# HKUST-Aerial-Robotics/Omni-swarm

Hardware: AMD Instinct MI355X
Metric: keyframes/sec (4x fisheye 600x480) + p50 loop-match ms @ 100k-frame DB (higher is better)
Workload: dtype f16

## Files before the change

### omni-swarm_amd/csrc/config.h

```cpp
#pragma once
#include "common.h"

namespace omni {

enum CfgId {
    CFG_CONV_V1 = 0, CFG_RS_TRN, CFG_DET16, CFG_SP_SPARSE_DESC, CFG_SP_SPARSE_DA, CFG_SP_FUSED_CAND, CFG_SP_SPLIT_DB, CFG_SP_MASK_SKIP, CFG_SP_MASK_SKIP_SPLIT, CFG_SP_MASK_RECT, CFG_SPLIT_FUSE1A, CFG_SPLIT_WINO,
    CFG_SPLIT_TRN, CFG_CONV_XCD, CFG_SP_PROFILE_MASK, CFG_PP_U8, CFG_PP_TRACE, CFG_PP_DBG, CFG_RS_TRACE, CFG_SPLIT_TRACE, CFG_SPLIT_DBG, CFG_WINO_TRACE, CFG_ROCTX,
    CFG_VLAD_BIG, CFG_VLAD_STEM_FUSE, CFG_VLAD_UNFUSED, CFG_VLAD_MFMA, CFG_VLAD_SBLOCK, CFG_VLAD_MBLOCK_PX, CFG_VLAD_MFMA_PX, CFG_VLAD_FC_MFMA, CFG_VLAD_MBLOCK_CPW,
    CFG_VLAD_SB_LDSPAD, CFG_VLAD_SB_PERSIST, CFG_VLAD_SB_TRACE, CFG_VLAD_SB_DBG, CFG_VLAD_MASK_SKIP,
    CFG_SCAN_ROWS_MIN, CFG_MQ_ROT, CFG_MQ_MIN, CFG_INDEX_MIRROR, CFG_INDEX_MIRROR_MIN_ROWS, CFG_INDEX_CERT_FAIL,
    CFG_GEOMETRY_THREADS, CFG_MESSAGE_THREADS, CFG_GEOMETRY_ASYNC, CFG_DETECTOR_ASYNC, CFG_PIPELINE_ONE_STREAM, CFG_PIPELINE_FIFO, CFG_PIPELINE_UNIT_PLAN,
    CFG_HW_QUEUES,
    CFG_RCCL_LIB,
    CFG_COUNT
};
enum CfgClass {
    CFG_VARIANT = 0,
    CFG_TUNING = 1,
    CFG_DEBUG = 2,
    CFG_TEST = 3,
    CFG_STRING = 4
};
struct CfgOption { const char* env; int def, lo, hi; int cls; const char* doc; };
extern const CfgOption kCfgOptions[CFG_COUNT];

struct Config {
    int v[CFG_COUNT];
    int operator[](CfgId i) const { return v[i]; }
};
int config_resolve(Config* out);
const Config& config_process();
int config_option_now(CfgId i);

}
```

### omni-swarm_amd/csrc/config.hip

```cpp
#include "config.h"

#include <atomic>
#include <cerrno>
#include <climits>
#include <cstdlib>

namespace omni {

const CfgOption kCfgOptions[CFG_COUNT] = {
    {"OMNI_CONV_V1", 0, 0, 3, CFG_VARIANT, "fp16 3x3 layers: 0 = production (conv1a fused into the ping-pong conv1b, register-stationary cin=128); 1 = generic kernel, 2 = persistent LDS-DMA kernel, "
                                           "3 = ping-pong without the conv1a fusion -- 1-3 exist only in the test build of the library (lib_test/)"},
    {"OMNI_RS_TRN", -1, -1, 1, CFG_VARIANT, "register-stationary kernel of the unpooled cin=128 fp16 layers: tile orientation, -1 = the one with fewer tiles, 0 = plain, 1 = transposed"},
    {"OMNI_DET16", 1, 0, 1, CFG_VARIANT, "detector head of the fp16 and OMNI_PREC_SPLIT paths on v_mfma_f32_32x32x16_f16 with split (hi, lo) operands (0: the exact-f32 MFMA kernel)"},
    {"OMNI_SP_SPARSE_DESC", 1, 0, 1, CFG_VARIANT, "convDb + descriptor norm only at the cells around the key points (0: dense descriptor map)"},
    {"OMNI_SP_SPARSE_DA", 1, 0, 1, CFG_VARIANT, "convDa only at those cells too (fp16 and OMNI_PREC_SPLIT; 0: dense convDa)"},
    {"OMNI_SP_FUSED_CAND", 1, 0, 1, CFG_VARIANT, "getKeyPoints' threshold inside the detector head's epilogue + window masks from the candidate list (0: sp_cand_kernel re-reads the heat map)"},
    {"OMNI_SP_SPLIT_DB", 1, 0, 1, CFG_VARIANT, "OMNI_PREC_SPLIT: convDb + descriptor norm at the key points' cells with split (hi, lo) operands on the fp16 matrix cores (0: exact-f32 MFMA convolution)"},
    {"OMNI_SP_MASK_SKIP", 1, 0, 1, CFG_VARIANT, "fp16: the tile rows inside the image-independent band of the fisheye mask are left out of the tile walk (0: every tile)"},
    {"OMNI_SP_MASK_SKIP_SPLIT", 1, 0, 1, CFG_VARIANT, "the same for OMNI_PREC_SPLIT"},
    {"OMNI_SP_MASK_RECT", 0, 0, 1, CFG_TEST, "1: a masked pass leaves out only the rectangle of tiles where the output is one constant vector, filled by broadcasting that vector "
                                             "(what was skipped before the band: the A/B reference, same results)"},
    {"OMNI_SPLIT_FUSE1A", 1, 0, 1, CFG_VARIANT, "OMNI_PREC_SPLIT: conv1a built inside the conv1b kernel from the u8 image (0: separate exact-f32 conv1a pass)"},
    {"OMNI_SPLIT_WINO", 7, 0, 15, CFG_VARIANT, "OMNI_PREC_SPLIT: the cin = 64 layers as Winograd F(2x2,3x3) kernels with split operands (conv_wino.hip), bit 0 = conv1b (with the conv1a "
                                                "fusion), 1 = conv2a, 2 = conv2b, 3 = conv3a (off by default: same time as the direct kernel, profiles/r06g); 0: the direct kernels of conv_split.hip"},
    {"OMNI_SPLIT_TRN", -1, -1, 1, CFG_VARIANT, "OMNI_PREC_SPLIT cin=128 kernel: tile orientation, as OMNI_RS_TRN"},
    {"OMNI_CONV_XCD", 1, 0, 1, CFG_VARIANT, "persistent convolution kernels derive (cout group, tile walk) from an XCD-aware block id: the cout groups of a pixel tile and its neighbours "
                                           "share one L2 (0: plain blockIdx; process-wide, same results either way)"},
    {"OMNI_SP_PROFILE_MASK", 0, 0, 1, CFG_TUNING, "omni_sp_profile times the stages with the fisheye mask on (what the key-frame pipeline runs)"},
    {"OMNI_PP_U8", 1, 0, 1, CFG_VARIANT, "fp16 conv1a inside conv1b's kernel: matrix-core operands straight from the image bytes (0: through the 256-entry u8 -> (hi, lo) table in LDS)"},
    {"OMNI_PP_TRACE", 0, 0, 1, CFG_DEBUG, "s_memtime trace of the ping-pong conv kernel on stderr"},
    {"OMNI_PP_DBG", 0, 0, 255, CFG_DEBUG, "ping-pong conv kernel timing ablations (WRONG results)"},
    {"OMNI_RS_TRACE", 0, 0, 1, CFG_DEBUG, "s_memtime trace of the register-stationary kernel"},
    {"OMNI_SPLIT_TRACE", 0, 0, 1, CFG_DEBUG, "s_memtime trace of the split-precision kernel"},
    {"OMNI_SPLIT_DBG", 0, 0, 3, CFG_DEBUG, "split-precision kernel timing ablations: 1 = no stores, 2 = every DMA reads tile 0 (WRONG results)"},
    {"OMNI_WINO_TRACE", 0, 0, 1, CFG_DEBUG, "s_memtime trace of the Winograd split kernel"},
    {"OMNI_ROCTX", 0, 0, 1, CFG_DEBUG, "roctx ranges around upload / SuperPoint / MobileNetVLAD / post-processing / BF match / index add + search / exchange and the host loop's "
                                      "stages (rocprofv3 --marker-trace; the library is resolved by dlopen)"},
    {"OMNI_VLAD_BIG", 0, 0, 128, CFG_TUNING, "64 / 128: the 64- / 128-pixel tiles of the unfused block kernel (measured slower at 600x480)"},
    {"OMNI_VLAD_STEM_FUSE", 1, 0, 1, CFG_VARIANT, "stem + block 0 in one kernel (0: two kernels)"},
    {"OMNI_VLAD_UNFUSED", 0, 0, 1, CFG_VARIANT, "1: every block as expand / depthwise / project launches"},
    {"OMNI_VLAD_MFMA", 1, 0, 1, CFG_VARIANT, "late blocks' 1x1 convolutions on the matrix cores"},
    {"OMNI_VLAD_SBLOCK", 1, 0, 1, CFG_VARIANT, "fused split-fp16 block kernel (vlad_s.hip)"},
    {"OMNI_VLAD_MBLOCK_PX", 2048, 0, 1 << 24, CFG_TUNING, "fused matrix-core block kernel for blocks of at most this many input pixels per image (0 disables)"},
    {"OMNI_VLAD_MFMA_PX", 0, 0, 1 << 24, CFG_TUNING, "> 0: matrix-core 1x1 convolutions for blocks of at most this many input pixels per image (default 2048)"},
    {"OMNI_VLAD_FC_MFMA", 1, 0, 1, CFG_VARIANT, "the final FC on the matrix cores (0: VALU kernel)"},
    {"OMNI_VLAD_MBLOCK_CPW", 0, 0, 64, CFG_TUNING, "hidden-layer split of the matrix-core block kernel: chunks per workgroup (0 = no split; measured: does not pay)"},
    {"OMNI_VLAD_SB_LDSPAD", 0, 0, 160 * 1024, CFG_DEBUG, "extra LDS bytes per workgroup of the split block kernel (occupancy A/B)"},
    {"OMNI_VLAD_SB_PERSIST", 1, 0, 16, CFG_VARIANT, "split block kernel: 0 = one tile per workgroup, N >= 1 = N x (CUs x resident workgroups) persistent workgroups"},
    {"OMNI_VLAD_SB_TRACE", 0, 0, 1, CFG_DEBUG, "s_memtime trace of the split block kernel"},
    {"OMNI_VLAD_SB_DBG", 0, 0, 255, CFG_DEBUG, "split block kernel timing ablations (WRONG results)"},
    {"OMNI_VLAD_MASK_SKIP", 1, 0, 1, CFG_VARIANT, "fisheye-masked passes leave the tiles of the first blocks that lie in the constant region of the mask out of the tile walk "
                                                  "(bit-identical; 0: the dense pass)"},
    {"OMNI_SCAN_ROWS_MIN", 4, 1, 1 << 20, CFG_TUNING, "fp32 scan: from this many queries on, the rows-stationary kernel"},
    {"OMNI_MQ_ROT", 1, 0, 1, CFG_VARIANT, "matrix-core multi-query scan: rotated query fragments"},
    {"OMNI_MQ_MIN", 4, 0, 1 << 20, CFG_TUNING, "queries from which an fp16 shard is searched on the matrix cores (1 = always, 0 = never)"},
    {"OMNI_INDEX_MIRROR", 1, 0, 1, CFG_VARIANT, "fp32 index: fp16 mirror + certificate for batched searches (0: exact scans only)"},
    {"OMNI_INDEX_MIRROR_MIN_ROWS", 32768, 0, INT_MAX, CFG_TUNING, "the mirror is used from this many rows on"},
    {"OMNI_INDEX_CERT_FAIL", 0, 0, 1, CFG_TEST, "1: every certificate fails (exercises the exact fallback)"},
    {"OMNI_GEOMETRY_THREADS", -1, -1, 1024, CFG_TUNING, "threads of the geometric-verification pool (-1: min(16, cores / 2); 0: inline)"},
    {"OMNI_MESSAGE_THREADS", 3, 0, 64, CFG_TUNING, "helper threads that fill a unit's key-frame messages (key points, descriptors, lifted points: ~75 KB per image, first-touch page "
                                                  "faults included) next to the calling thread while the unit's detector step runs on the GPU (0: inline)"},
    {"OMNI_GEOMETRY_ASYNC", 1, 0, 1, CFG_VARIANT, "a micro-batch's geometry tasks run while the next unit is waited for (0: drained at once)"},
    {"OMNI_DETECTOR_ASYNC", 1, 0, 1, CFG_VARIANT, "a micro-batch's detector step (appends, searches) is enqueued and collected one unit later (0: the host waits for it on the spot)"},
    {"OMNI_PIPELINE_ONE_STREAM", 0, 0, 1, CFG_VARIANT, "a unit's MobileNetVLAD launches behind its SuperPoint launches on one stream (0: next to them on a second stream)"},
    {"OMNI_PIPELINE_FIFO", -1, -1, 2, CFG_VARIANT, "units in flight run oldest first: a unit's SuperPoint stream (1) / both its streams (2) start behind the convolution stack of the unit "
                                                   "enqueued before it; 0: the units' kernels take turns; -1: by measurement -- 1 for the fp32-class precisions, whose time is all "
                                                   "CU-filling convolutions (+2-4 %), and for an fp16 run() of no more units than lanes (all in flight at once: +13 % at 3 units), 0 for fp16 otherwise, whose small-grid "
                                                   "tails the next units' kernels fill (-5 % when chained)"},
    {"OMNI_PIPELINE_UNIT_PLAN", 1, 0, 2, CFG_VARIANT, "KeyframePipeline::run on host blocks, a run that is not a whole number of micro-batches: 1 = units of equal size (20 key frames = "
                                                       "7 + 7 + 6), 2 = the same behind half a unit, 0 = the blocks' own cut (8 + 8 + 4)"},
    {"OMNI_HW_QUEUES", 8, 0, 64, CFG_TUNING, "hardware queues asked of the HIP runtime when the library is loaded (GPU_MAX_HW_QUEUES, unless already set): the pipeline's five "
                                            "streams must not share one; 0 = the runtime's default of 4"},
    {"OMNI_RCCL_LIB", 0, 0, 0, CFG_STRING, "path of the RCCL library omni_shard dlopens (default: librccl.so next to torch, then the loader's search path)"},
};

static int parse_one(const CfgOption& o, int* out, bool* bad) {
    *out = o.def; *bad = false;
    if (o.cls == CFG_STRING) return 0;
    const char* e = getenv(o.env);
    if (!e || !e[0]) return 0;
    errno = 0;
    char* end = nullptr;
    const long v = strtol(e, &end, 10);
    if (errno || end == e || *end != '\0' || v < o.lo || v > o.hi) { *bad = true; return 0; }
    *out = (int)v;
    return 1;
}

int config_resolve(Config* out) {
    for (int i = 0; i < CFG_COUNT; ++i) {
        bool bad;
        parse_one(kCfgOptions[i], &out->v[i], &bad);
        OMNI_REQUIRE(!bad, OMNI_ERR_INVALID, "%s=%s: expected an integer in [%d, %d] (%s)", kCfgOptions[i].env, getenv(kCfgOptions[i].env), kCfgOptions[i].lo, kCfgOptions[i].hi,
                     kCfgOptions[i].doc);
    }
    return OMNI_OK;
}

static bool is_process_wide(int i) {
    switch (i) {
        case CFG_CONV_XCD: case CFG_INDEX_CERT_FAIL: case CFG_INDEX_MIRROR: case CFG_INDEX_MIRROR_MIN_ROWS: case CFG_MQ_ROT:
        case CFG_PP_DBG: case CFG_PP_TRACE: case CFG_RS_TRACE: case CFG_RS_TRN: case CFG_SCAN_ROWS_MIN: case CFG_SPLIT_DBG: case CFG_SPLIT_TRACE: case CFG_SPLIT_TRN: case CFG_WINO_TRACE: case CFG_ROCTX:
        case CFG_VLAD_BIG: case CFG_VLAD_SB_DBG: case CFG_VLAD_SB_LDSPAD: case CFG_VLAD_SB_TRACE:
            return true;
        default:
            return false;
    }
}
static std::atomic<bool> g_process_resolved{false};

int config_option_now(CfgId i) {
    int v; bool bad;
    parse_one(kCfgOptions[i], &v, &bad);
    return v;
}

const Config& config_process() {
    static const Config c = [] {
        g_process_resolved.store(true);
        Config q;
        for (int i = 0; i < CFG_COUNT; ++i) {
            bool bad;
            parse_one(kCfgOptions[i], &q.v[i], &bad);
            if (bad) fprintf(stderr, "libomni_hip: %s=%s ignored: expected an integer in [%d, %d]\n", kCfgOptions[i].env, getenv(kCfgOptions[i].env), kCfgOptions[i].lo, kCfgOptions[i].hi);
        }
        return q;
    }();
    return c;
}

}

extern "C" {

int omni_config_count(void) { return omni::CFG_COUNT; }

int omni_config_describe(int i, const char** env, int* def, int* lo, int* hi, int* cls, const char** doc) {
    OMNI_REQUIRE(i >= 0 && i < omni::CFG_COUNT, OMNI_ERR_INVALID, "omni_config_describe: option %d of %d", i, (int)omni::CFG_COUNT);
    const omni::CfgOption& o = omni::kCfgOptions[i];
    if (env) *env = o.env;
    if (def) *def = o.def;
    if (lo) *lo = o.lo;
    if (hi) *hi = o.hi;
    if (cls) *cls = o.cls;
    if (doc) *doc = o.doc;
    return OMNI_OK;
}

int omni_config_is_process_wide(int i) { return (i >= 0 && i < omni::CFG_COUNT && omni::is_process_wide(i)) ? 1 : 0; }

int omni_config_value(const char* env, int* value) {
    OMNI_REQUIRE(env && value, OMNI_ERR_INVALID, "null argument");
    omni::Config c;
    const int rc = omni::config_resolve(&c);
    if (rc) return rc;
    for (int i = 0; i < omni::CFG_COUNT; ++i)
        if (!strcmp(omni::kCfgOptions[i].env, env)) {
            *value = (omni::is_process_wide(i) && omni::g_process_resolved.load()) ? omni::config_process()[(omni::CfgId)i] : c.v[i];
            return OMNI_OK;
        }
    omni::set_error("omni_config_value: no option named %s", env);
    return OMNI_ERR_INVALID;
}

}
```

### omni-swarm_amd/csrc/vlad_s.hip

```cpp
#include "config.h"
#include "common.h"
#include "vlad_h.h"
#include "vlad_plan.h"

namespace omni {

typedef _Float16 sh8 __attribute__((ext_vector_type(8)));
typedef _Float16 sh4 __attribute__((ext_vector_type(4)));
typedef _Float16 sh2 __attribute__((ext_vector_type(2)));
typedef float sf16 __attribute__((ext_vector_type(16)));
typedef float sf2 __attribute__((ext_vector_type(2)));
typedef float sf4 __attribute__((ext_vector_type(4)));

#define SB_CH 48
#define SB_HS 208
#define SB_DS 112
#define SB_WD (10 * SB_CH)

__device__ __forceinline__ int sb_div(int n, unsigned m) { return m ? (int)__umulhi((unsigned)n, m) : n; }

template <int STRIDE, int CIN, int NT>
struct SBlockCfg {
    static constexpr int S1 = (2 * CIN + 2 + 15) / 16, S2 = (CIN + 15) / 16;
    static constexpr int XS = S1 * 32 + 16;
    static constexpr int TH = vlad_sblock_th(STRIDE), OPX = 8 * TH, NTN = OPX / 32;
    static_assert(VLAD_SBLOCK_TW == 8, "the tiles of vlad_sblock_kernel are 8 pixels wide");
    static constexpr int RWX = 7 * STRIDE + 3, RHY = (TH - 1) * STRIDE + 3, R = RWX * RHY, RT = (R + 31) / 32, RP = RT * 32;
    static constexpr int NW = RT < 4 ? RT : 4, THREADS = NW * 64, XP = (R + THREADS / 2 - 1) / (THREADS / 2);
    static constexpr int CB = (S1 + S2) * 2048 + NT * 6144;
    static constexpr int MQ = STRIDE == 1 ? (NT + 1) / 2 : 1;
    static constexpr size_t smem(int hid) { return (size_t)R * XS + 2 * (size_t)OPX * SB_DS + (size_t)R * SB_HS + (size_t)(hid / SB_CH) * SB_WD * 4; }
};

#ifndef SB_WPE_SMALL
#define SB_WPE_SMALL 2
#endif
template <int STRIDE, int CIN, int NT>
__global__ void __launch_bounds__((SBlockCfg<STRIDE, CIN, NT>::THREADS), (CIN > 32 ? 1 : (CIN <= 16 ? SB_WPE_SMALL : 2)))
vlad_sblock_kernel(VladSBlockArgs a) {
    using C = SBlockCfg<STRIDE, CIN, NT>;
    constexpr int S1 = C::S1, S2 = C::S2, XS = C::XS, TH = C::TH, OPX = C::OPX, RWX = C::RWX, R = C::R, CB = C::CB, MQ = C::MQ, NW = C::NW, RT = C::RT, XP = C::XP;
    extern __shared__ __attribute__((aligned(16))) char smem[];
    const int n_chunks = a.hid / SB_CH;
    char* xin = smem;
    char* dhi = smem + R * XS;
    char* dlo = dhi + OPX * SB_DS;
    char* h = dlo + OPX * SB_DS;
    float* wdl = reinterpret_cast<float*>(h + R * SB_HS);
    const int tid = threadIdx.x, lane = tid & 63, wave = __builtin_amdgcn_readfirstlane(tid >> 6);
    const int n = lane & 31, kk = lane >> 5;
    const int tiles_x = (a.Wo + 7) >> 3, tiles_y = (a.Ho + TH - 1) / TH, tiles_img = tiles_x * tiles_y;
    const char* blob = reinterpret_cast<const char*>(a.blob);
    const char* frag = blob + (size_t)n_chunks * SB_WD * 4;

    sh8 we1[S1][2], we2[S2][2];
    auto load_we = [&](int c) {
        const char* cb = frag + (int64_t)c * CB + lane * 16;
#pragma unroll
        for (int ks = 0; ks < S1; ++ks)
#pragma unroll
            for (int m = 0; m < 2; ++m) we1[ks][m] = *reinterpret_cast<const sh8*>(cb + (ks * 2 + m) * 1024);
#pragma unroll
        for (int ks = 0; ks < S2; ++ks)
#pragma unroll
            for (int m = 0; m < 2; ++m) we2[ks][m] = *reinterpret_cast<const sh8*>(cb + ((S1 + ks) * 2 + m) * 1024);
    };
    load_we(0);
    {
        const sf4* ws = reinterpret_cast<const sf4*>(blob);
        for (int e = tid; e < n_chunks * (SB_WD / 4); e += C::THREADS) reinterpret_cast<sf4*>(wdl)[e] = ws[e];
    }
    const int pair = tid % 24, blk = tid / 24;
    const int nt = STRIDE == 1 ? (wave & 1) : 0;
    const int mt0 = STRIDE == 1 ? (wave >> 1) : wave;
    constexpr int MSTEP = STRIDE == 1 ? 2 : NW;
    const bool pwave = mt0 < NT;
    sf4 pbias[MQ][4];
#pragma unroll
    for (int q = 0; q < MQ; ++q)
#pragma unroll
        for (int g = 0; g < 4; ++g) {
            const int ch = (mt0 + MSTEP * q) * 32 + 8 * g + 4 * kk;
            const sf4 z = {0.f, 0.f, 0.f, 0.f};
            pbias[q][g] = ch < a.cout ? *reinterpret_cast<const sf4*>(a.bp + ch) : z;
        }

    auto tile_origin = [&](int tile, int& tb, int& toy, int& tox) {
        tb = sb_div(tile, a.m_img);
        const int ttr = tile - tb * tiles_img, tty = sb_div(ttr, a.m_tx);
        toy = tty * TH; tox = (ttr - tty * tiles_x) * 8;
    };
    const int act_total = a.walk.act * a.batch;
    auto full_tile = [&](int t) -> int {
        if (a.walk.y1 <= a.walk.y0) return t;
        const int tb = sb_div(t, a.m_act);
        return tb * tiles_img + tile_walk_index(a.walk, tiles_x, t - tb * a.walk.act);
    };
    const int xhf = tid & 1;
    sf4 xpre[XP][CIN / 8];
    bool xin_img[XP];
    auto fetch_x = [&](int tile) {
        int tb, toy, tox;
        tile_origin(tile, tb, toy, tox);
#pragma unroll
        for (int ps = 0; ps < XP; ++ps) {
            const int xr = (tid >> 1) + ps * (C::THREADS / 2), xry = xr / RWX, xrx = xr - xry * RWX;
            const int gy = toy * STRIDE - 1 + xry, gx = tox * STRIDE - 1 + xrx;
            xin_img[ps] = xr < R && gy >= 0 && gy < a.Hi && gx >= 0 && gx < a.Wi;
            const unsigned off = (unsigned)((tb * a.Hi + gy) * a.Wi + gx) * CIN + xhf * (CIN / 2);
#pragma unroll
            for (int q = 0; q < CIN / 8; ++q) {
                const sf4 z = {0.f, 0.f, 0.f, 0.f};
                xpre[ps][q] = xin_img[ps] ? *reinterpret_cast<const sf4*>(a.in + off + q * 4) : z;
            }
        }
    };
    sf16 acc[MQ];
    sf4 resv[MQ][4];
    unsigned out_off = 0;
    bool out_ok = false;
    auto out_pixel = [&](int tile, unsigned& off_out, unsigned& off_res) {
        int tb, toy, tox;
        tile_origin(tile, tb, toy, tox);
        const int o = nt * 32 + n, oy = toy + (o >> 3), ox = tox + (o & 7);
        off_out = (unsigned)((tb * a.Ho + oy) * a.Wo + ox) * (unsigned)a.cout;
        off_res = (unsigned)((tb * a.Hi + oy) * a.Wi + ox) * (unsigned)CIN;
        return pwave && oy < a.Ho && ox < a.Wo;
    };
    auto fetch_res = [&](bool ok, unsigned off_res) {
        if (!a.res) return;
#pragma unroll
        for (int q = 0; q < MQ; ++q)
#pragma unroll
            for (int g = 0; g < 4; ++g) {
                const int ch = (mt0 + MSTEP * q) * 32 + 8 * g + 4 * kk;
                const sf4 z = {0.f, 0.f, 0.f, 0.f};
                resv[q][g] = (ok && ch < a.cout) ? *reinterpret_cast<const sf4*>(a.in + off_res + ch) : z;
            }
    };
    auto store_out = [&]() {
        if (!out_ok || (a.dbg & 1)) return;
#pragma unroll
        for (int q = 0; q < MQ; ++q)
#pragma unroll
            for (int g = 0; g < 4; ++g) {
                const int ch = (mt0 + MSTEP * q) * 32 + 8 * g + 4 * kk;
                if (ch >= a.cout) continue;
                sf4 v = pbias[q][g];
#pragma unroll
                for (int j = 0; j < 4; ++j) v[j] += acc[q][4 * g + j];
                if (a.res) v += resv[q][g];
                *reinterpret_cast<sf4*>(a.out + out_off + ch) = v;
            }
    };

    auto expand = [&]() {
#pragma unroll
      for (int rt = 0; rt < (RT + NW - 1) / NW; ++rt) {
        const int rw = wave + rt * NW;
        if (rw >= RT) break;
        const char* xb = xin + (rw * 32 + n) * XS + kk * 16;
        sf16 e0, e1;
#pragma unroll
        for (int r = 0; r < 16; ++r) { e0[r] = 0.f; e1[r] = 0.f; }
#pragma unroll
        for (int ks = 0; ks < S1; ++ks) {
            const sh8 xb8 = *reinterpret_cast<const sh8*>(xb + ks * 32);
            e0 = __builtin_amdgcn_mfma_f32_32x32x16_f16(we1[ks][0], xb8, e0, 0, 0, 0);
            e1 = __builtin_amdgcn_mfma_f32_32x32x16_f16(we1[ks][1], xb8, e1, 0, 0, 0);
        }
#pragma unroll
        for (int ks = 0; ks < S2; ++ks) {
            const sh8 xb8 = *reinterpret_cast<const sh8*>(xb + ks * 32);
            e0 = __builtin_amdgcn_mfma_f32_32x32x16_f16(we2[ks][0], xb8, e0, 0, 0, 0);
            e1 = __builtin_amdgcn_mfma_f32_32x32x16_f16(we2[ks][1], xb8, e1, 0, 0, 0);
        }
        if (rw * 32 + n < R) {
            char* hp = h + (rw * 32 + n) * SB_HS + kk * 16;
#pragma unroll
            for (int g = 0; g < 4; ++g) {
                sf4 v;
#pragma unroll
                for (int j = 0; j < 4; ++j) v[j] = __builtin_amdgcn_fmed3f(e0[4 * g + j], 0.f, 6.f);
                *reinterpret_cast<sf4*>(hp + g * 32) = v;
            }
#pragma unroll
            for (int g = 0; g < 2; ++g) {
                sf4 v;
#pragma unroll
                for (int j = 0; j < 4; ++j) v[j] = __builtin_amdgcn_fmed3f(e1[4 * g + j], 0.f, 6.f);
                *reinterpret_cast<sf4*>(hp + 128 + g * 32) = v;
            }
        }
      }
    };

    if ((int)blockIdx.x < act_total) fetch_x(full_tile(blockIdx.x));
#define TR(k) do { if (trw) a.trace[wave * 16 + (k)] = __builtin_amdgcn_s_memtime(); } while (0)
    for (int t = blockIdx.x; t < act_total; t += gridDim.x) {
        const int tile = full_tile(t);
        const bool trw = a.trace && blockIdx.x == 0 && (tid & 63) == 0 && t == (int)blockIdx.x + 2 * (int)gridDim.x;
        TR(8);
#pragma unroll
        for (int ps = 0; ps < XP; ++ps) {
            const int xr = (tid >> 1) + ps * (C::THREADS / 2);
            if (xr < R) {
                char* row = xin + xr * XS;
#pragma unroll
                for (int q = 0; q < CIN / 8; ++q) {
                    const sf4 v = xpre[ps][q];
                    const sh4 hi = __builtin_convertvector(v, sh4);
                    const sh4 lo = __builtin_convertvector(v - __builtin_convertvector(hi, sf4), sh4);
                    *reinterpret_cast<sh4*>(row + (xhf * (CIN / 2) + q * 4) * 2) = hi;
                    *reinterpret_cast<sh4*>(row + CIN * 2 + (xhf * (CIN / 2) + q * 4) * 2) = lo;
                }
                sh8 t = {0, 0, 0, 0, 0, 0, 0, 0};
                if (xhf == 0 && xin_img[ps]) { t[0] = (_Float16)1.f; t[1] = (_Float16)1.f; }
                *reinterpret_cast<sh8*>(row + CIN * 4 + xhf * 16) = t;
            }
        }
        store_out();
        {
            unsigned off_res;
            out_ok = out_pixel(tile, out_off, off_res);
            fetch_res(out_ok, off_res);
        }
        if (t + (int)gridDim.x < act_total && !(a.dbg & 2)) fetch_x(full_tile(t + gridDim.x));
#pragma unroll
        for (int p = 0; p < MQ; ++p)
#pragma unroll
            for (int r = 0; r < 16; ++r) acc[p][r] = 0.f;

        __syncthreads();
        TR(0);
        expand();
        TR(1);
        __syncthreads();
        TR(2);

        for (int c = 0; c < n_chunks; ++c) {
            const char* cb = frag + (int64_t)c * CB + (S1 + S2) * 2048 + lane * 16;
            sh8 wph[MQ][3], wpl[MQ][3];
#pragma unroll
            for (int q = 0; q < MQ; ++q) {
                const int m = mt0 + MSTEP * q;
#pragma unroll
                for (int ks = 0; ks < 3; ++ks) {
                    const sh8 z = {0, 0, 0, 0, 0, 0, 0, 0};
                    wph[q][ks] = m < NT ? *reinterpret_cast<const sh8*>(cb + ((m * 3 + ks) * 2 + 0) * 1024) : z;
                    wpl[q][ks] = m < NT ? *reinterpret_cast<const sh8*>(cb + ((m * 3 + ks) * 2 + 1) * 1024) : z;
                }
            }
            if (n_chunks > 1) load_we(c + 1 < n_chunks ? c + 1 : 0);
            if (tid < 192) {
                const float* wd = wdl + c * SB_WD + pair * 2;
                sf2 w9[9];
#pragma unroll
                for (int t = 0; t < 9; ++t) w9[t] = *reinterpret_cast<const sf2*>(wd + t * SB_CH);
                const sf2 bias = *reinterpret_cast<const sf2*>(wd + 9 * SB_CH);
                constexpr int BW = STRIDE == 1 ? 4 : 2, BH = 2;
                constexpr int IW = (BW - 1) * STRIDE + 3, IH = (BH - 1) * STRIDE + 3;
                const int by = STRIDE == 1 ? (blk >> 1) : (blk >> 2), bx = STRIDE == 1 ? (blk & 1) * 4 : (blk & 3) * 2;
                const char* hp = h + ((by * BH * STRIDE) * RWX + bx * STRIDE) * SB_HS + pair * 8;
                sf2 v[IH][IW];
#pragma unroll
                for (int y = 0; y < IH; ++y)
#pragma unroll
                    for (int x = 0; x < IW; ++x) v[y][x] = *reinterpret_cast<const sf2*>(hp + (y * RWX + x) * SB_HS);
#pragma unroll
                for (int oy = 0; oy < BH; ++oy)
#pragma unroll
                    for (int ox = 0; ox < BW; ++ox) {
                        sf2 o = bias;
#pragma unroll
                        for (int dy = 0; dy < 3; ++dy)
#pragma unroll
                            for (int dx = 0; dx < 3; ++dx) o = __builtin_elementwise_fma(v[oy * STRIDE + dy][ox * STRIDE + dx], w9[dy * 3 + dx], o);
                        sf2 r; r[0] = __builtin_amdgcn_fmed3f(o[0], 0.f, 6.f); r[1] = __builtin_amdgcn_fmed3f(o[1], 0.f, 6.f);
                        const sh2 hi = __builtin_convertvector(r, sh2);
                        const sh2 lo = __builtin_convertvector(r - __builtin_convertvector(hi, sf2), sh2);
                        const int off = ((by * BH + oy) * 8 + bx + ox) * SB_DS + pair * 4;
                        *reinterpret_cast<sh2*>(dhi + off) = hi;
                        *reinterpret_cast<sh2*>(dlo + off) = lo;
                    }
            }
            TR(3);
            __syncthreads();
            TR(4);
            if (pwave) {
                const int doff = (nt * 32 + n) * SB_DS + kk * 16;
                sh8 bh[3], bl[3];
#pragma unroll
                for (int ks = 0; ks < 3; ++ks) {
                    bh[ks] = *reinterpret_cast<const sh8*>(dhi + doff + ks * 32);
                    bl[ks] = *reinterpret_cast<const sh8*>(dlo + doff + ks * 32);
                }
#pragma unroll
                for (int q = 0; q < MQ; ++q) {
                    if (mt0 + MSTEP * q < NT) {
#pragma unroll
                        for (int ks = 0; ks < 3; ++ks) {
                            acc[q] = __builtin_amdgcn_mfma_f32_32x32x16_f16(wph[q][ks], bh[ks], acc[q], 0, 0, 0);
                            acc[q] = __builtin_amdgcn_mfma_f32_32x32x16_f16(wph[q][ks], bl[ks], acc[q], 0, 0, 0);
                            acc[q] = __builtin_amdgcn_mfma_f32_32x32x16_f16(wpl[q][ks], bh[ks], acc[q], 0, 0, 0);
                        }
                    }
                }
            }
            TR(5);
            if (c + 1 < n_chunks) {
                expand();
                __syncthreads();
            }
            TR(6);
        }
        TR(7);
    }
#undef TR
    store_out();
}

static inline uint16_t sb_f2h(float v) { const __half hv = __float2half_rn(v); uint16_t u; memcpy(&u, &hv, 2); return u; }
static inline float sb_h2f(uint16_t u) { __half hv; memcpy(&hv, &u, 2); return __half2float(hv); }
static inline float sb_hi(float v) { return sb_h2f(sb_f2h(v)); }
static inline float sb_lo(float v) { return v - sb_hi(v); }

#define SB_SHAPES(X) X(2, 8, 1) X(1, 8, 1) X(1, 16, 1) X(2, 16, 1) X(1, 24, 1) X(1, 32, 1) X(2, 32, 2) X(1, 56, 2) X(1, 56, 4)

bool vlad_sblock_supported(int cin, int hid, int cout, int stride) {
    if (hid < SB_CH || hid % SB_CH || cout % 4 || cout < 4) return false;
    const int nt0 = (cout + 31) / 32, nt = nt0 == 3 ? 4 : nt0;
#define X(S, CI, N) if (stride == S && cin == CI && nt == N) return true;
    SB_SHAPES(X)
#undef X
    return false;
}

static inline int sb_nt(int cout) { const int nt0 = (cout + 31) / 32; return nt0 == 3 ? 4 : nt0; }

size_t vlad_sblock_blob_bytes(int cin, int hid, int cout) {
    const int S1 = (2 * cin + 2 + 15) / 16, S2 = (cin + 15) / 16, NT = sb_nt(cout);
    return (size_t)(hid / SB_CH) * (SB_WD * 4 + (S1 + S2) * 2048 + NT * 6144);
}

void vlad_sblock_pack(int cin, int hid, int cout, const float* we, const float* be, const float* wd, const float* bd, const float* wp, void* out) {
    const int S1 = (2 * cin + 2 + 15) / 16, S2 = (cin + 15) / 16, NT = sb_nt(cout), CB = (S1 + S2) * 2048 + NT * 6144;
    const int n_chunks = hid / SB_CH;
    memset(out, 0, vlad_sblock_blob_bytes(cin, hid, cout));
    float* wdo = reinterpret_cast<float*>(out);
    for (int ch = 0; ch < hid; ++ch) {
        float* q = wdo + (size_t)(ch / SB_CH) * SB_WD + ch % SB_CH;
        for (int t = 0; t < 9; ++t) q[t * SB_CH] = wd[(size_t)ch * 9 + t];
        q[9 * SB_CH] = bd[ch];
    }
    char* frag = reinterpret_cast<char*>(out) + (size_t)n_chunks * SB_WD * 4;
    for (int c = 0; c < n_chunks; ++c) {
        char* cb = frag + (size_t)c * CB;
        for (int pass = 0; pass < 2; ++pass)
            for (int ks = 0; ks < (pass ? S2 : S1); ++ks)
                for (int m = 0; m < 2; ++m)
                    for (int l = 0; l < 64; ++l)
                        for (int e = 0; e < 8; ++e) {
                            const int row = m * 32 + (l & 31), k = ks * 16 + (l >> 5) * 8 + e;
                            float v = 0.f;
                            if (row < SB_CH) {
                                const int ch = c * SB_CH + row;
                                if (!pass) {
                                    if (k < cin) v = sb_hi(we[(size_t)ch * cin + k]);
                                    else if (k < 2 * cin) v = sb_hi(we[(size_t)ch * cin + k - cin]);
                                    else if (k == 2 * cin) v = sb_hi(be[ch]);
                                    else if (k == 2 * cin + 1) v = sb_lo(be[ch]);
                                } else if (k < cin) v = sb_lo(we[(size_t)ch * cin + k]);
                            }
                            reinterpret_cast<uint16_t*>(cb + (((pass ? S1 : 0) + ks) * 2 + m) * 1024)[l * 8 + e] = sb_f2h(v);
                        }
        for (int m = 0; m < NT; ++m)
            for (int ks = 0; ks < 3; ++ks)
                for (int part = 0; part < 2; ++part)
                    for (int l = 0; l < 64; ++l)
                        for (int e = 0; e < 8; ++e) {
                            const int co = m * 32 + (l & 31), hc = c * SB_CH + ks * 16 + (l >> 5) * 8 + e;
                            float v = 0.f;
                            if (co < cout) v = part ? sb_lo(wp[(size_t)co * hid + hc]) : sb_hi(wp[(size_t)co * hid + hc]);
                            reinterpret_cast<uint16_t*>(cb + (S1 + S2) * 2048 + ((m * 3 + ks) * 2 + part) * 1024)[l * 8 + e] = sb_f2h(v);
                        }
    }
}

template <int STRIDE, int CIN, int NT>
static int launch_sb(hipStream_t st, const VladSBlockArgs& a) {
    using C = SBlockCfg<STRIDE, CIN, NT>;
    static const size_t pad = (size_t)config_process()[CFG_VLAD_SB_LDSPAD];
    const size_t smem = C::smem(a.hid) + pad;
    OMNI_REQUIRE(smem <= 160 * 1024, OMNI_ERR_CAPACITY, "vlad_sblock: %zu B of LDS for hid=%d", smem, a.hid);
    auto kfn = vlad_sblock_kernel<STRIDE, CIN, NT>;
    static DynSmemState attr;
    OMNI_HIP_TRY(ensure_dyn_smem(attr, (const void*)kfn, smem));
    const int tiles_x = cdiv(a.Wo, 8), tiles_y = cdiv(a.Ho, C::TH);
    VladSBlockArgs at = a;
    if (int rc = tile_walk_plan(at.walk, "vlad_sblock", tiles_x, tiles_y, a.sk_y0, a.sk_y1, a.sk_x0, a.sk_x0 + a.sk_w)) return rc;
    const int tiles = at.walk.act * a.batch;
    OMNI_REQUIRE((int64_t)a.batch * a.Hi * a.Wi * a.cin < (1ll << 31) && (int64_t)a.batch * a.Ho * a.Wo * a.cout < (1ll << 31) && tiles < (1 << 20),
                 OMNI_ERR_CAPACITY, "vlad_sblock: tensor beyond 32-bit element offsets");
    static int per_cu_cached = 0;
    static size_t per_cu_smem = 0;
    if (!per_cu_cached || per_cu_smem != smem) {
        int nb = 0;
        OMNI_HIP_TRY(hipOccupancyMaxActiveBlocksPerMultiprocessor(&nb, (const void*)kfn, C::THREADS, smem));
        per_cu_cached = nb < 1 ? 1 : nb;
        per_cu_smem = smem;
    }
    const int per_cu = per_cu_cached;
    const int persist = a.persist;
    const int64_t cap = (int64_t)a.n_cu * per_cu * (persist > 0 ? persist : 1);
    const int grid = (!persist || tiles < cap) ? tiles : (int)cap;
    static const bool want_trace = config_process()[CFG_VLAD_SB_TRACE] != 0;
    static unsigned long long* trace_dev = nullptr;
    at.trace = nullptr;
    static const int dbg = config_process()[CFG_VLAD_SB_DBG];
    at.dbg = dbg;
    at.m_img = tile_walk_magic(tiles_x * tiles_y);
    at.m_tx = tile_walk_magic(tiles_x);
    at.m_act = tile_walk_magic(at.walk.act);
    if (want_trace) {
        if (!trace_dev) OMNI_HIP_TRY(hipMalloc((void**)&trace_dev, 8 * 16 * 8));
        OMNI_HIP_TRY(hipMemsetAsync(trace_dev, 0, 8 * 16 * 8, st));
        at.trace = trace_dev;
    }
    hipLaunchKernelGGL(kfn, dim3(grid), dim3(C::THREADS), smem, st, at);
    OMNI_LAUNCH_CHECK();
    if (want_trace) {
        unsigned long long hbuf[8 * 16];
        OMNI_HIP_TRY(hipMemcpyAsync(hbuf, trace_dev, sizeof(hbuf), hipMemcpyDeviceToHost, st));
        OMNI_HIP_TRY(hipStreamSynchronize(st));
        static int launches = 0;
        if (launches++ == 8)
            for (int w = 0; w < C::THREADS / 64; ++w) {
                const unsigned long long* t = hbuf + w * 16;
                if (!t[8]) continue;
                fprintf(stderr, "sb trace s%d cin%d grid %d wave %d (last chunk): x->lds+store+bar %llu expand %llu bar %llu | dw %llu bar %llu proj %llu | tile %llu\n",
                        STRIDE, CIN, grid, w, t[0] - t[8], t[1] - t[0], t[2] - t[1], t[3] - t[2], t[4] - t[3], t[5] - t[4], t[7] - t[8]);
            }
    }
    return OMNI_OK;
}

int launch_vlad_sblock(hipStream_t st, const VladSBlockArgs& a, int stride) {
    const int nt = sb_nt(a.cout);
#define X(S, CI, N) if (stride == S && a.cin == CI && nt == N) return launch_sb<S, CI, N>(st, a);
    SB_SHAPES(X)
#undef X
    set_error("vlad_sblock: no instantiation for cin=%d cout=%d stride=%d", a.cin, a.cout, stride);
    return OMNI_ERR_INVALID;
}

}
```

Measured before the change: 2737.

## Stage split-block weight fragments in LDS once per workgroup and chunk

In the fused split-fp16 block kernel, each wave used to load the expand and projection weight fragments straight from global memory into registers for every chunk. Now the workgroup fetches each fragment once, cooperatively, prefetching the next chunk's fragments while the depthwise step runs, and stores them in LDS. The MFMA loops then read their operands from LDS. The launcher picks LDS-staged modes only when occupancy does not drop, which trades extra LDS traffic and footprint for fewer global loads and lower register pressure. A test-only grid cap option is added as well.

```diff
diff --git a/omni-swarm_amd/csrc/config.h b/omni-swarm_amd/csrc/config.h
--- a/omni-swarm_amd/csrc/config.h
+++ b/omni-swarm_amd/csrc/config.h
@@ -7,7 +7,7 @@
     CFG_CONV_V1 = 0, CFG_RS_TRN, CFG_DET16, CFG_SP_SPARSE_DESC, CFG_SP_SPARSE_DA, CFG_SP_FUSED_CAND, CFG_SP_SPLIT_DB, CFG_SP_MASK_SKIP, CFG_SP_MASK_SKIP_SPLIT, CFG_SP_MASK_RECT, CFG_SPLIT_FUSE1A, CFG_SPLIT_WINO,
     CFG_SPLIT_TRN, CFG_CONV_XCD, CFG_SP_PROFILE_MASK, CFG_PP_U8, CFG_PP_TRACE, CFG_PP_DBG, CFG_RS_TRACE, CFG_SPLIT_TRACE, CFG_SPLIT_DBG, CFG_WINO_TRACE, CFG_ROCTX,
     CFG_VLAD_BIG, CFG_VLAD_STEM_FUSE, CFG_VLAD_UNFUSED, CFG_VLAD_MFMA, CFG_VLAD_SBLOCK, CFG_VLAD_MBLOCK_PX, CFG_VLAD_MFMA_PX, CFG_VLAD_FC_MFMA, CFG_VLAD_MBLOCK_CPW,
-    CFG_VLAD_SB_LDSPAD, CFG_VLAD_SB_PERSIST, CFG_VLAD_SB_TRACE, CFG_VLAD_SB_DBG, CFG_VLAD_MASK_SKIP,
+    CFG_VLAD_SB_LDSPAD, CFG_VLAD_SB_PERSIST, CFG_VLAD_SB_TRACE, CFG_VLAD_SB_DBG, CFG_VLAD_SB_WREG, CFG_VLAD_SB_GRID, CFG_VLAD_MASK_SKIP,
     CFG_SCAN_ROWS_MIN, CFG_MQ_ROT, CFG_MQ_MIN, CFG_INDEX_MIRROR, CFG_INDEX_MIRROR_MIN_ROWS, CFG_INDEX_CERT_FAIL,
     CFG_GEOMETRY_THREADS, CFG_MESSAGE_THREADS, CFG_GEOMETRY_ASYNC, CFG_DETECTOR_ASYNC, CFG_PIPELINE_ONE_STREAM, CFG_PIPELINE_FIFO, CFG_PIPELINE_UNIT_PLAN,
     CFG_HW_QUEUES,
diff --git a/omni-swarm_amd/csrc/config.hip b/omni-swarm_amd/csrc/config.hip
--- a/omni-swarm_amd/csrc/config.hip
+++ b/omni-swarm_amd/csrc/config.hip
@@ -49,6 +49,9 @@
     {"OMNI_VLAD_SB_PERSIST", 1, 0, 16, CFG_VARIANT, "split block kernel: 0 = one tile per workgroup, N >= 1 = N x (CUs x resident workgroups) persistent workgroups"},
     {"OMNI_VLAD_SB_TRACE", 0, 0, 1, CFG_DEBUG, "s_memtime trace of the split block kernel"},
     {"OMNI_VLAD_SB_DBG", 0, 0, 255, CFG_DEBUG, "split block kernel timing ablations (WRONG results)"},
+    {"OMNI_VLAD_SB_WREG", 0, 0, 2, CFG_TEST, "split block kernel, blocks of more than one hidden chunk: 1 = every wave fetches the matrix fragments it multiplies by into registers "
+                                             "(the form before they were staged in LDS once per workgroup and chunk: the A/B reference, same results); 2 = only the projection fragments"},
+    {"OMNI_VLAD_SB_GRID", 0, 0, 1 << 20, CFG_TEST, "split block kernel: at most this many workgroups per launch (0: no cap), so that a small map makes every workgroup walk several tiles"},
     {"OMNI_VLAD_MASK_SKIP", 1, 0, 1, CFG_VARIANT, "fisheye-masked passes leave the tiles of the first blocks that lie in the constant region of the mask out of the tile walk "
                                                   "(bit-identical; 0: the dense pass)"},
     {"OMNI_SCAN_ROWS_MIN", 4, 1, 1 << 20, CFG_TUNING, "fp32 scan: from this many queries on, the rows-stationary kernel"},
@@ -101,7 +104,7 @@
     switch (i) {
         case CFG_CONV_XCD: case CFG_INDEX_CERT_FAIL: case CFG_INDEX_MIRROR: case CFG_INDEX_MIRROR_MIN_ROWS: case CFG_MQ_ROT:
         case CFG_PP_DBG: case CFG_PP_TRACE: case CFG_RS_TRACE: case CFG_RS_TRN: case CFG_SCAN_ROWS_MIN: case CFG_SPLIT_DBG: case CFG_SPLIT_TRACE: case CFG_SPLIT_TRN: case CFG_WINO_TRACE: case CFG_ROCTX:
-        case CFG_VLAD_BIG: case CFG_VLAD_SB_DBG: case CFG_VLAD_SB_LDSPAD: case CFG_VLAD_SB_TRACE:
+        case CFG_VLAD_BIG: case CFG_VLAD_SB_DBG: case CFG_VLAD_SB_LDSPAD: case CFG_VLAD_SB_TRACE: case CFG_VLAD_SB_WREG: case CFG_VLAD_SB_GRID:
             return true;
         default:
             return false;
diff --git a/omni-swarm_amd/csrc/vlad_s.hip b/omni-swarm_amd/csrc/vlad_s.hip
--- a/omni-swarm_amd/csrc/vlad_s.hip
+++ b/omni-swarm_amd/csrc/vlad_s.hip
@@ -29,31 +29,42 @@
     static constexpr int NW = RT < 4 ? RT : 4, THREADS = NW * 64, XP = (R + THREADS / 2 - 1) / (THREADS / 2);
     static constexpr int CB = (S1 + S2) * 2048 + NT * 6144;
     static constexpr int MQ = STRIDE == 1 ? (NT + 1) / 2 : 1;
-    static constexpr size_t smem(int hid) { return (size_t)R * XS + 2 * (size_t)OPX * SB_DS + (size_t)R * SB_HS + (size_t)(hid / SB_CH) * SB_WD * 4; }
+    static constexpr int NFE = (S1 + S2) * 2, NFP = NT * 6;
+    static constexpr size_t smem(int hid, int wmode = 0) {
+        return (size_t)R * XS + 2 * (size_t)OPX * SB_DS + (size_t)R * SB_HS + (size_t)(hid / SB_CH) * SB_WD * 4 + (wmode >= 1 ? NFE * 1024 : 0) + (wmode >= 2 ? NFP * 1024 : 0);
+    }
+    static constexpr int WG_CU = CIN > 32 ? 1 : 2;
+    static constexpr int lds_wgs(size_t bytes) { return (int)(160 * 1024 / bytes) < WG_CU ? (int)(160 * 1024 / bytes) : WG_CU; }
+    static constexpr bool STAGED = CIN > 8 && lds_wgs(smem(6 * CIN, 1)) >= lds_wgs(smem(6 * CIN, 0));
+    static constexpr bool PFIT = STAGED && lds_wgs(smem(6 * CIN, 2)) >= lds_wgs(smem(6 * CIN, 0));
 };
 
 #ifndef SB_WPE_SMALL
 #define SB_WPE_SMALL 2
 #endif
-template <int STRIDE, int CIN, int NT>
+template <int STRIDE, int CIN, int NT, int WMODE>
 __global__ void __launch_bounds__((SBlockCfg<STRIDE, CIN, NT>::THREADS), (CIN > 32 ? 1 : (CIN <= 16 ? SB_WPE_SMALL : 2)))
 vlad_sblock_kernel(VladSBlockArgs a) {
     using C = SBlockCfg<STRIDE, CIN, NT>;
     constexpr int S1 = C::S1, S2 = C::S2, XS = C::XS, TH = C::TH, OPX = C::OPX, RWX = C::RWX, R = C::R, CB = C::CB, MQ = C::MQ, NW = C::NW, RT = C::RT, XP = C::XP;
+    constexpr bool ES = WMODE >= 1, PS = WMODE >= 2;
+    constexpr int NFE = C::NFE, NFP = C::NFP, QE = (NFE + NW - 1) / NW, QP = (NFP + NW - 1) / NW;
     extern __shared__ __attribute__((aligned(16))) char smem[];
     const int n_chunks = a.hid / SB_CH;
     char* xin = smem;
     char* dhi = smem + R * XS;
     char* dlo = dhi + OPX * SB_DS;
     char* h = dlo + OPX * SB_DS;
-    float* wdl = reinterpret_cast<float*>(h + R * SB_HS);
+    char* wel = h + R * SB_HS;
+    char* wpq = wel + (ES ? NFE * 1024 : 0);
+    float* wdl = reinterpret_cast<float*>(wpq + (PS ? NFP * 1024 : 0));
     const int tid = threadIdx.x, lane = tid & 63, wave = __builtin_amdgcn_readfirstlane(tid >> 6);
     const int n = lane & 31, kk = lane >> 5;
     const int tiles_x = (a.Wo + 7) >> 3, tiles_y = (a.Ho + TH - 1) / TH, tiles_img = tiles_x * tiles_y;
     const char* blob = reinterpret_cast<const char*>(a.blob);
     const char* frag = blob + (size_t)n_chunks * SB_WD * 4;
 
-    sh8 we1[S1][2], we2[S2][2];
+    sh8 we1[ES ? 1 : S1][2], we2[ES ? 1 : S2][2];
     auto load_we = [&](int c) {
         const char* cb = frag + (int64_t)c * CB + lane * 16;
 #pragma unroll
@@ -65,7 +76,33 @@
 #pragma unroll
             for (int m = 0; m < 2; ++m) we2[ks][m] = *reinterpret_cast<const sh8*>(cb + ((S1 + ks) * 2 + m) * 1024);
     };
-    load_we(0);
+    sh8 sge[ES ? QE : 1], sgp[PS ? QP : 1];
+    const int so = tid * 16;
+    auto sg_mine = [&](int i, int nf) { return (i + 1) * NW <= nf || so + i * NW * 1024 < nf * 1024; };
+    auto stage_fetch_e = [&](int c) {
+        const char* cb = frag + (int64_t)c * CB + so;
+#pragma unroll
+        for (int i = 0; i < QE; ++i)
+            if (sg_mine(i, NFE)) sge[i] = *reinterpret_cast<const sh8*>(cb + i * NW * 1024);
+    };
+    auto stage_put_e = [&]() {
+#pragma unroll
+        for (int i = 0; i < QE; ++i)
+            if (sg_mine(i, NFE)) *reinterpret_cast<sh8*>(wel + so + i * NW * 1024) = sge[i];
+    };
+    auto stage_fetch_p = [&](int c) {
+        const char* cb = frag + (int64_t)c * CB + NFE * 1024 + so;
+#pragma unroll
+        for (int i = 0; i < QP; ++i)
+            if (sg_mine(i, NFP)) sgp[i] = *reinterpret_cast<const sh8*>(cb + i * NW * 1024);
+    };
+    auto stage_put_p = [&]() {
+#pragma unroll
+        for (int i = 0; i < QP; ++i)
+            if (sg_mine(i, NFP)) *reinterpret_cast<sh8*>(wpq + so + i * NW * 1024) = sgp[i];
+    };
+    if constexpr (ES) { stage_fetch_e(0); stage_put_e(); }
+    else load_we(0);
     {
         const sf4* ws = reinterpret_cast<const sf4*>(blob);
         for (int e = tid; e < n_chunks * (SB_WD / 4); e += C::THREADS) reinterpret_cast<sf4*>(wdl)[e] = ws[e];
@@ -154,6 +191,10 @@
             }
     };
 
+    auto wfrag = [&](int ks, int m) -> sh8 {
+        if constexpr (ES) return *reinterpret_cast<const sh8*>(wel + (ks * 2 + m) * 1024 + lane * 16);
+        else return ks < S1 ? we1[ks][m] : we2[ks - S1][m];
+    };
     auto expand = [&]() {
 #pragma unroll
       for (int rt = 0; rt < (RT + NW - 1) / NW; ++rt) {
@@ -166,14 +207,14 @@
 #pragma unroll
         for (int ks = 0; ks < S1; ++ks) {
             const sh8 xb8 = *reinterpret_cast<const sh8*>(xb + ks * 32);
-            e0 = __builtin_amdgcn_mfma_f32_32x32x16_f16(we1[ks][0], xb8, e0, 0, 0, 0);
-            e1 = __builtin_amdgcn_mfma_f32_32x32x16_f16(we1[ks][1], xb8, e1, 0, 0, 0);
+            e0 = __builtin_amdgcn_mfma_f32_32x32x16_f16(wfrag(ks, 0), xb8, e0, 0, 0, 0);
+            e1 = __builtin_amdgcn_mfma_f32_32x32x16_f16(wfrag(ks, 1), xb8, e1, 0, 0, 0);
         }
 #pragma unroll
         for (int ks = 0; ks < S2; ++ks) {
             const sh8 xb8 = *reinterpret_cast<const sh8*>(xb + ks * 32);
-            e0 = __builtin_amdgcn_mfma_f32_32x32x16_f16(we2[ks][0], xb8, e0, 0, 0, 0);
-            e1 = __builtin_amdgcn_mfma_f32_32x32x16_f16(we2[ks][1], xb8, e1, 0, 0, 0);
+            e0 = __builtin_amdgcn_mfma_f32_32x32x16_f16(wfrag(S1 + ks, 0), xb8, e0, 0, 0, 0);
+            e1 = __builtin_amdgcn_mfma_f32_32x32x16_f16(wfrag(S1 + ks, 1), xb8, e1, 0, 0, 0);
         }
         if (rw * 32 + n < R) {
             char* hp = h + (rw * 32 + n) * SB_HS + kk * 16;
@@ -240,18 +281,23 @@
 
         for (int c = 0; c < n_chunks; ++c) {
             const char* cb = frag + (int64_t)c * CB + (S1 + S2) * 2048 + lane * 16;
-            sh8 wph[MQ][3], wpl[MQ][3];
-#pragma unroll
-            for (int q = 0; q < MQ; ++q) {
-                const int m = mt0 + MSTEP * q;
-#pragma unroll
-                for (int ks = 0; ks < 3; ++ks) {
-                    const sh8 z = {0, 0, 0, 0, 0, 0, 0, 0};
-                    wph[q][ks] = m < NT ? *reinterpret_cast<const sh8*>(cb + ((m * 3 + ks) * 2 + 0) * 1024) : z;
-                    wpl[q][ks] = m < NT ? *reinterpret_cast<const sh8*>(cb + ((m * 3 + ks) * 2 + 1) * 1024) : z;
+            sh8 wph[PS ? 1 : MQ][3], wpl[PS ? 1 : MQ][3];
+            const int c_next = c + 1 < n_chunks ? c + 1 : 0;
+            if constexpr (PS) stage_fetch_p(c);
+            if constexpr (ES) { if (n_chunks > 1) stage_fetch_e(c_next); }
+            if constexpr (!PS) {
+#pragma unroll
+                for (int q = 0; q < MQ; ++q) {
+                    const int m = mt0 + MSTEP * q;
+#pragma unroll
+                    for (int ks = 0; ks < 3; ++ks) {
+                        const sh8 z = {0, 0, 0, 0, 0, 0, 0, 0};
+                        wph[q][ks] = m < NT ? *reinterpret_cast<const sh8*>(cb + ((m * 3 + ks) * 2 + 0) * 1024) : z;
+                        wpl[q][ks] = m < NT ? *reinterpret_cast<const sh8*>(cb + ((m * 3 + ks) * 2 + 1) * 1024) : z;
+                    }
                 }
             }
-            if (n_chunks > 1) load_we(c + 1 < n_chunks ? c + 1 : 0);
+            if constexpr (!ES) { if (n_chunks > 1) load_we(c_next); }
             if (tid < 192) {
                 const float* wd = wdl + c * SB_WD + pair * 2;
                 sf2 w9[9];
@@ -284,6 +330,8 @@
                         *reinterpret_cast<sh2*>(dlo + off) = lo;
                     }
             }
+            if constexpr (PS) stage_put_p();
+            if constexpr (ES) { if (n_chunks > 1) stage_put_e(); }
             TR(3);
             __syncthreads();
             TR(4);
@@ -297,12 +345,18 @@
                 }
 #pragma unroll
                 for (int q = 0; q < MQ; ++q) {
-                    if (mt0 + MSTEP * q < NT) {
+                    const int m = mt0 + MSTEP * q;
+                    if (m < NT) {
 #pragma unroll
                         for (int ks = 0; ks < 3; ++ks) {
-                            acc[q] = __builtin_amdgcn_mfma_f32_32x32x16_f16(wph[q][ks], bh[ks], acc[q], 0, 0, 0);
-                            acc[q] = __builtin_amdgcn_mfma_f32_32x32x16_f16(wph[q][ks], bl[ks], acc[q], 0, 0, 0);
-                            acc[q] = __builtin_amdgcn_mfma_f32_32x32x16_f16(wpl[q][ks], bh[ks], acc[q], 0, 0, 0);
+                            sh8 ph, pl;
+                            if constexpr (PS) {
+                                ph = *reinterpret_cast<const sh8*>(wpq + ((m * 3 + ks) * 2 + 0) * 1024 + lane * 16);
+                                pl = *reinterpret_cast<const sh8*>(wpq + ((m * 3 + ks) * 2 + 1) * 1024 + lane * 16);
+                            } else { ph = wph[q][ks]; pl = wpl[q][ks]; }
+                            acc[q] = __builtin_amdgcn_mfma_f32_32x32x16_f16(ph, bh[ks], acc[q], 0, 0, 0);
+                            acc[q] = __builtin_amdgcn_mfma_f32_32x32x16_f16(ph, bl[ks], acc[q], 0, 0, 0);
+                            acc[q] = __builtin_amdgcn_mfma_f32_32x32x16_f16(pl, bh[ks], acc[q], 0, 0, 0);
                         }
                     }
                 }
@@ -387,21 +441,15 @@
     }
 }
 
-template <int STRIDE, int CIN, int NT>
-static int launch_sb(hipStream_t st, const VladSBlockArgs& a) {
+template <int STRIDE, int CIN, int NT, int WMODE>
+static int sb_resident(int hid, size_t* smem_out, int* per_cu) {
     using C = SBlockCfg<STRIDE, CIN, NT>;
     static const size_t pad = (size_t)config_process()[CFG_VLAD_SB_LDSPAD];
-    const size_t smem = C::smem(a.hid) + pad;
-    OMNI_REQUIRE(smem <= 160 * 1024, OMNI_ERR_CAPACITY, "vlad_sblock: %zu B of LDS for hid=%d", smem, a.hid);
-    auto kfn = vlad_sblock_kernel<STRIDE, CIN, NT>;
+    const size_t smem = C::smem(hid, WMODE) + pad;
+    OMNI_REQUIRE(smem <= 160 * 1024, OMNI_ERR_CAPACITY, "vlad_sblock: %zu B of LDS for hid=%d", smem, hid);
+    auto kfn = vlad_sblock_kernel<STRIDE, CIN, NT, WMODE>;
     static DynSmemState attr;
     OMNI_HIP_TRY(ensure_dyn_smem(attr, (const void*)kfn, smem));
-    const int tiles_x = cdiv(a.Wo, 8), tiles_y = cdiv(a.Ho, C::TH);
-    VladSBlockArgs at = a;
-    if (int rc = tile_walk_plan(at.walk, "vlad_sblock", tiles_x, tiles_y, a.sk_y0, a.sk_y1, a.sk_x0, a.sk_x0 + a.sk_w)) return rc;
-    const int tiles = at.walk.act * a.batch;
-    OMNI_REQUIRE((int64_t)a.batch * a.Hi * a.Wi * a.cin < (1ll << 31) && (int64_t)a.batch * a.Ho * a.Wo * a.cout < (1ll << 31) && tiles < (1 << 20),
-                 OMNI_ERR_CAPACITY, "vlad_sblock: tensor beyond 32-bit element offsets");
     static int per_cu_cached = 0;
     static size_t per_cu_smem = 0;
     if (!per_cu_cached || per_cu_smem != smem) {
@@ -410,10 +458,29 @@
         per_cu_cached = nb < 1 ? 1 : nb;
         per_cu_smem = smem;
     }
-    const int per_cu = per_cu_cached;
+    *smem_out = smem;
+    *per_cu = per_cu_cached;
+    return OMNI_OK;
+}
+
+template <int STRIDE, int CIN, int NT, int WMODE>
+static int launch_sb_mode(hipStream_t st, const VladSBlockArgs& a) {
+    using C = SBlockCfg<STRIDE, CIN, NT>;
+    size_t smem = 0;
+    int per_cu = 1;
+    if (int rc = sb_resident<STRIDE, CIN, NT, WMODE>(a.hid, &smem, &per_cu)) return rc;
+    auto kfn = vlad_sblock_kernel<STRIDE, CIN, NT, WMODE>;
+    const int tiles_x = cdiv(a.Wo, 8), tiles_y = cdiv(a.Ho, C::TH);
+    VladSBlockArgs at = a;
+    if (int rc = tile_walk_plan(at.walk, "vlad_sblock", tiles_x, tiles_y, a.sk_y0, a.sk_y1, a.sk_x0, a.sk_x0 + a.sk_w)) return rc;
+    const int tiles = at.walk.act * a.batch;
+    OMNI_REQUIRE((int64_t)a.batch * a.Hi * a.Wi * a.cin < (1ll << 31) && (int64_t)a.batch * a.Ho * a.Wo * a.cout < (1ll << 31) && tiles < (1 << 20),
+                 OMNI_ERR_CAPACITY, "vlad_sblock: tensor beyond 32-bit element offsets");
     const int persist = a.persist;
     const int64_t cap = (int64_t)a.n_cu * per_cu * (persist > 0 ? persist : 1);
-    const int grid = (!persist || tiles < cap) ? tiles : (int)cap;
+    static const int grid_cap = config_process()[CFG_VLAD_SB_GRID];
+    int grid = (!persist || tiles < cap) ? tiles : (int)cap;
+    if (grid_cap > 0 && grid > grid_cap) grid = grid_cap;
     static const bool want_trace = config_process()[CFG_VLAD_SB_TRACE] != 0;
     static unsigned long long* trace_dev = nullptr;
     at.trace = nullptr;
@@ -438,11 +505,39 @@
             for (int w = 0; w < C::THREADS / 64; ++w) {
                 const unsigned long long* t = hbuf + w * 16;
                 if (!t[8]) continue;
-                fprintf(stderr, "sb trace s%d cin%d grid %d wave %d (last chunk): x->lds+store+bar %llu expand %llu bar %llu | dw %llu bar %llu proj %llu | tile %llu\n",
-                        STRIDE, CIN, grid, w, t[0] - t[8], t[1] - t[0], t[2] - t[1], t[3] - t[2], t[4] - t[3], t[5] - t[4], t[7] - t[8]);
+                fprintf(stderr, "sb trace s%d cin%d nt%d wmode %d lds %zu per-cu %d grid %d wave %d (last chunk): x->lds+store+bar %llu expand %llu bar %llu | dw %llu bar %llu proj %llu | tile %llu\n",
+                        STRIDE, CIN, NT, WMODE, smem, per_cu, grid, w, t[0] - t[8], t[1] - t[0], t[2] - t[1], t[3] - t[2], t[4] - t[3], t[5] - t[4], t[7] - t[8]);
             }
     }
     return OMNI_OK;
+}
+
+template <int STRIDE, int CIN, int NT>
+static int launch_sb(hipStream_t st, const VladSBlockArgs& a) {
+    using C = SBlockCfg<STRIDE, CIN, NT>;
+    if constexpr (C::STAGED) {
+        static const int wreg = config_process()[CFG_VLAD_SB_WREG];
+        static int mode = -1;
+        if (mode < 0) {
+            int m = 0, r0 = 0, r1 = 0, r2 = 0;
+            size_t bytes;
+            if (wreg != 1) {
+                if (int rc = sb_resident<STRIDE, CIN, NT, 0>(a.hid, &bytes, &r0)) return rc;
+                if (int rc = sb_resident<STRIDE, CIN, NT, 1>(a.hid, &bytes, &r1)) return rc;
+                if (r1 >= r0) m = 1;
+                if constexpr (C::PFIT) {
+                    if (m == 1 && wreg == 0) {
+                        if (int rc = sb_resident<STRIDE, CIN, NT, 2>(a.hid, &bytes, &r2)) return rc;
+                        if (r2 >= r0) m = 2;
+                    }
+                }
+            }
+            mode = m;
+        }
+        if constexpr (C::PFIT) { if (mode == 2) return launch_sb_mode<STRIDE, CIN, NT, 2>(st, a); }
+        if (mode == 1) return launch_sb_mode<STRIDE, CIN, NT, 1>(st, a);
+    }
+    return launch_sb_mode<STRIDE, CIN, NT, 0>(st, a);
 }
 
 int launch_vlad_sblock(hipStream_t st, const VladSBlockArgs& a, int stride) {
```

New measurement: 2735. Within noise of the previous version (-0.1%).
